# kanyu369/ADNM-UNet

Hardware: AMD Instinct MI355X
Metric: sequences/sec training ADNM-UNet 5->20x128x128 (higher is better)
Workload: dtype bf16; 1 GPU; ADNM-UNet create_ADNMUNet(5,20,6) 128x128 full training step (fwd + enRainfallLoss + bwd + clip_grad_norm_ + AdamW), recipe parameters, synthetic radar frames in HBM; per_gpu_batch=4, global_batch=4, frames=5->20, parallelism=single, launch=hipGraph replay

## Files before the change

### adnm-unet_amd/csrc/planar.hip

```cpp
#include "adnm_common.h"

namespace {

constexpr int kBlock = 256;

__device__ __forceinline__ float4 f4zero() { return make_float4(0.f, 0.f, 0.f, 0.f); }

template <typename T, int CX>
__global__ __launch_bounds__(kBlock) void haar_dwt_kernel(const T* __restrict__ x, int64_t ldx, T* __restrict__ y, int B, int H,
                                                          int W, int C) {
  const int C4 = C >> 2, h2 = (H + 1) >> 1, w2 = (W + 1) >> 1;
  const int64_t total = (int64_t)B * h2 * w2 * C4;
  const int64_t idx = (int64_t)blockIdx.x * kBlock + threadIdx.x;
  if (idx >= total) return;
  const int cg = (int)(idx % C4);
  int64_t t = idx / C4;
  const int j = (int)(t % w2);
  t /= w2;
  const int i = (int)(t % h2);
  const int b = (int)(t / h2);
  float v[4][4];
#pragma unroll
  for (int q = 0; q < 4; ++q) {
    const int hh = 2 * i + (q >> 1), ww = 2 * j + (q & 1);
// ... 348 lines not shown
                                                                    int cgb, int ppc, int act) {
  __shared__ __attribute__((aligned(16))) float smem[3 * 2 * 64 * 4];
  const int C4 = C >> 2;
  const int cgl = threadIdx.x & (cgb - 1), slot = threadIdx.x / cgb, slots = kBlock / cgb;
  const int cg = blockIdx.x * cgb + cgl;
  const bool cv = cg < C4;
  const int c = cv ? cg * 4 : 0;
  const int b = blockIdx.z;
  const T* xb = x + (int64_t)b * HW * C + c;
  const T* db = dy + (int64_t)b * HW * C + c;
  const float4 mu = *reinterpret_cast<const float4*>(mu_in + (int64_t)b * C + c);
  const float4 rs = *reinterpret_cast<const float4*>(rstd_in + (int64_t)b * C + c);
  const float sc = scale ? *scale : 1.f, sh = shift ? *shift : 0.f;
  float4 acc[2] = {f4zero(), f4zero()};
  const int64_t p0 = (int64_t)blockIdx.y * ppc;
  const int64_t p1 = p0 + ppc < HW ? p0 + ppc : HW;
  if (cv)
    for (int64_t p = p0 + slot; p < p1; p += slots) {
      const float4 v = Io<T>::ld4(xb + p * C), g = Io<T>::ld4(db + p * C);
      const float4 xh = make_float4((v.x - mu.x) * rs.x, (v.y - mu.y) * rs.y, (v.z - mu.z) * rs.z, (v.w - mu.w) * rs.w);
      const float4 ag = actg4(make_float4(sc * xh.x + sh, sc * xh.y + sh, sc * xh.z + sh, sc * xh.w + sh), act);
      const float4 dp = make_float4(g.x * ag.x, g.y * ag.y, g.z * ag.z, g.w * ag.w);
      acc[0].x += dp.x; acc[0].y += dp.y; acc[0].z += dp.z; acc[0].w += dp.w;
      acc[1].x = fmaf(dp.x, xh.x, acc[1].x); acc[1].y = fmaf(dp.y, xh.y, acc[1].y);
      acc[1].z = fmaf(dp.z, xh.z, acc[1].z); acc[1].w = fmaf(dp.w, xh.w, acc[1].w);
    }
  fold_slots<2>(acc, cgb, smem);
  if ((threadIdx.x >> 6) == 0) {
    const bool mine = (threadIdx.x & 63) < cgb && cv;
    if (mine) {
      float* dst = part + ((int64_t)b * gridDim.y + blockIdx.y) * 2 * C;
      *reinterpret_cast<float4*>(dst + c) = acc[0];
      *reinterpret_cast<float4*>(dst + C + c) = acc[1];
    }
    if (spart) {
      float a = mine ? (acc[0].x + acc[0].y) + (acc[0].z + acc[0].w) : 0.f, q = mine ? (acc[1].x + acc[1].y) + (acc[1].z + acc[1].w) : 0.f;
      a = wave_sum(a), q = wave_sum(q);
      if (threadIdx.x == 0) {
        float* sp = spart + (((int64_t)b * gridDim.y + blockIdx.y) * gridDim.x + blockIdx.x) * 2;
        sp[0] = a, sp[1] = q;
      }
    }
  }
}

template <typename T>
__global__ __launch_bounds__(kBlock) void instnorm_bwd_apply_kernel(const T* __restrict__ dy, const T* __restrict__ x,
                                                                    const float* __restrict__ part, const float* __restrict__ scale,
                                                                    const float* __restrict__ shift, const float* __restrict__ mu_in,
                                                                    const float* __restrict__ rstd_in, T* __restrict__ dx, int64_t HW,
                                                                    int C, int cgb, int ppc, int nchunk, int act) {
  const int C4 = C >> 2;
  const int cgl = threadIdx.x & (cgb - 1), slot = threadIdx.x / cgb, slots = kBlock / cgb;
  const int cg = blockIdx.x * cgb + cgl;
  const bool cv = cg < C4;
  const int c = cv ? cg * 4 : 0;
  const int b = blockIdx.z;
  float4 s1, s2;
  merge_partials(part, b, nchunk, C, c, cv, cgb, s1, s2);
  if (!cv) return;
  const T* xb = x + (int64_t)b * HW * C + c;
  const T* db = dy + (int64_t)b * HW * C + c;
  T* ob = dx + (int64_t)b * HW * C + c;
  const float4 mu = *reinterpret_cast<const float4*>(mu_in + (int64_t)b * C + c);
  const float4 rs = *reinterpret_cast<const float4*>(rstd_in + (int64_t)b * C + c);
  const float sc = scale ? *scale : 1.f, sh = shift ? *shift : 0.f;
  const float inv = 1.0f / (float)HW;
  s1.x *= inv; s1.y *= inv; s1.z *= inv; s1.w *= inv;
  s2.x *= inv; s2.y *= inv; s2.z *= inv; s2.w *= inv;
  const int64_t p0 = (int64_t)blockIdx.y * ppc;
  const int64_t p1 = p0 + ppc < HW ? p0 + ppc : HW;
  for (int64_t p = p0 + slot; p < p1; p += slots) {
    const float4 v = Io<T>::ld4(xb + p * C), g = Io<T>::ld4(db + p * C);
    const float4 xh = make_float4((v.x - mu.x) * rs.x, (v.y - mu.y) * rs.y, (v.z - mu.z) * rs.z, (v.w - mu.w) * rs.w);
    const float4 ag = actg4(make_float4(sc * xh.x + sh, sc * xh.y + sh, sc * xh.z + sh, sc * xh.w + sh), act);
    float4 o;
    o.x = rs.x * sc * (g.x * ag.x - s1.x - xh.x * s2.x);
    o.y = rs.y * sc * (g.y * ag.y - s1.y - xh.y * s2.y);
    o.z = rs.z * sc * (g.z * ag.z - s1.z - xh.z * s2.z);
    o.w = rs.w * sc * (g.w * ag.w - s1.w - xh.w * s2.w);
    Io<T>::st4(ob + p * C, o);
  }
}



__device__ __forceinline__ float hsum4(float4 v) { return (v.x + v.y) + (v.z + v.w); }
__device__ __forceinline__ float dot4(float4 a, float4 b) { return (a.x * b.x + a.y * b.y) + (a.z * b.z + a.w * b.w); }
__device__ __forceinline__ float4 ld4_or(const float* p, int c, float dflt) {
  return p ? *reinterpret_cast<const float4*>(p + c) : make_float4(dflt, dflt, dflt, dflt);
}

__device__ __forceinline__ void group_sums(float h1, float h2, const float* __restrict__ part, const float* __restrict__ w, int b,
                                           int nchunk, int C, int c, bool cv, int cgb, int cpg, float& g1, float& g2) {
  __shared__ float gsm[2][64];
  if (threadIdx.x < cgb) gsm[0][threadIdx.x] = h1, gsm[1][threadIdx.x] = h2;
  __syncthreads();
  g1 = g2 = 0.f;
  if (!cv) return;
  const int qpg = cpg >> 2, q0 = c / cpg * qpg, base = blockIdx.x * cgb;
  if (q0 >= base && q0 + qpg <= base + cgb) {
    for (int q = q0 - base; q < q0 - base + qpg; ++q) g1 += gsm[0][q], g2 += gsm[1][q];
  } else {
    for (int q = q0; q < q0 + qpg; ++q) {
      float4 a = f4zero(), s = f4zero();
      for (int k = 0; k < nchunk; ++k) {
        const float* src = part + ((int64_t)b * nchunk + k) * 2 * C + q * 4;
        const float4 ak = *reinterpret_cast<const float4*>(src), sk = *reinterpret_cast<const float4*>(src + C);
        a.x += ak.x; a.y += ak.y; a.z += ak.z; a.w += ak.w;
        s.x += sk.x; s.y += sk.y; s.z += sk.z; s.w += sk.w;
      }
      const float4 wq = ld4_or(w, q * 4, 1.f);
      g1 += dot4(wq, a), g2 += dot4(wq, s);
    }
  }
}

template <typename T>
__global__ __launch_bounds__(kBlock) void groupnorm_apply_kernel(const T* __restrict__ x, const float* __restrict__ part,
                                                                 const float* __restrict__ gamma, const float* __restrict__ beta,
                                                                 const float* __restrict__ scale, const float* __restrict__ shift,
                                                                 T* __restrict__ y, float* __restrict__ mu_out, float* __restrict__ rstd_out,
                                                                 int64_t HW, int C, int cpg, int cgb, int ppc, int nchunk, float eps, int act) {
  const int C4 = C >> 2;
  const int cgl = threadIdx.x & (cgb - 1), slot = threadIdx.x / cgb, slots = kBlock / cgb;
  const int cg = blockIdx.x * cgb + cgl;
  const bool cv = cg < C4;
  const int c = cv ? cg * 4 : 0;
  const int b = blockIdx.z;
  float4 s1, s2;
  merge_partials(part, b, nchunk, C, c, cv, cgb, s1, s2);
  float g1, g2;
  group_sums(hsum4(s1), hsum4(s2), part, nullptr, b, nchunk, C, c, cv, cgb, cpg, g1, g2);
  if (!cv) return;
  const T* xb = x + (int64_t)b * HW * C + c;
  T* yb = y + (int64_t)b * HW * C + c;
  const float K = Io<T>::ld(xb - c % cpg);
  const float inv = 1.0f / ((float)HW * (float)cpg);
  const float m = g1 * inv;
  const float rstd = rsqrtf(fmaxf(g2 * inv - m * m, 0.f) + eps);
  if (blockIdx.y == 0 && slot == 0 && c % cpg == 0) {
    const int64_t at = (int64_t)b * (C / cpg) + c / cpg;
    mu_out[at] = K + m;
    rstd_out[at] = rstd;
  }
  const float sc = scale ? *scale : 1.f, sh = shift ? *shift : 0.f;
  const float4 ga = ld4_or(gamma, c, 1.f), be = ld4_or(beta, c, 0.f);
  const float4 a = make_float4(sc * ga.x * rstd, sc * ga.y * rstd, sc * ga.z * rstd, sc * ga.w * rstd);
  const float4 o0 = make_float4(fmaf(sc, be.x, sh), fmaf(sc, be.y, sh), fmaf(sc, be.z, sh), fmaf(sc, be.w, sh));
  const int64_t p0 = (int64_t)blockIdx.y * ppc;
  const int64_t p1 = p0 + ppc < HW ? p0 + ppc : HW;
  for (int64_t p = p0 + slot; p < p1; p += slots) {
    const float4 v = Io<T>::ld4(xb + p * C);
    float4 o = make_float4(fmaf((v.x - K) - m, a.x, o0.x), fmaf((v.y - K) - m, a.y, o0.y), fmaf((v.z - K) - m, a.z, o0.z),
                           fmaf((v.w - K) - m, a.w, o0.w));
    Io<T>::st4(yb + p * C, act4(o, act));
  }
}

template <typename T>
__global__ __launch_bounds__(kBlock) void groupnorm_bwd_stats_kernel(const T* __restrict__ dy, const T* __restrict__ x,
                                                                     const float* __restrict__ gamma, const float* __restrict__ beta,
                                                                     const float* __restrict__ scale, const float* __restrict__ shift,
                                                                     const float* __restrict__ mu_in, const float* __restrict__ rstd_in,
                                                                     float* __restrict__ part, float* __restrict__ spart, int64_t HW, int C,
                                                                     int cpg, int cgb, int ppc, int act) {
// ... 110 lines not shown

extern "C" int adnm_haar_idwt(const void* s, const void* up1, const void* up2, const void* ll_add, const void* y_add1, const void* y_add2, void* y,
                              int64_t B, int64_t H, int64_t W, int64_t C, int dtype, adnm_stream_t stream) {
  ADNM_REQUIRE(s && y, "haar_idwt: null pointer");
  ADNM_REQUIRE(up1 || !up2, "haar_idwt: the coarser levels must be filled in order (up2 without up1)");
  ADNM_REQUIRE(B > 0 && H > 0 && W > 0 && C > 0 && C % 4 == 0, "haar_idwt: bad shape (C=%lld must be a multiple of 4)", (long long)C);
  ADNM_REQUIRE(dtype == ADNM_F32 || dtype == ADNM_BF16, "haar_idwt: bad dtype %d", dtype);
  const int64_t total = B * ((H + 1) / 2) * ((W + 1) / 2) * (C / 4);
  const unsigned grid = (unsigned)adnm_cdiv(total, kBlock);
  hipStream_t st = (hipStream_t)stream;
  const double units = 2.0 + (up1 ? 0.25 : 0.0) + (up2 ? 0.0625 : 0.0) + (ll_add ? (up2 ? 0.015625 : (up1 ? 0.0625 : 0.25)) : 0.0) + (y_add1 ? 1.0 : 0.0) + (y_add2 ? 1.0 : 0.0);
  const int up = up2 ? 2 : (up1 ? 1 : 0);
#define IDWT(T, UP) haar_idwt_kernel<T, UP><<<grid, kBlock, 0, st>>>((const T*)s, (const T*)up1, (const T*)up2, (const T*)ll_add, (const T*)y_add1, (const T*)y_add2, (T*)y, (int)B, (int)H, (int)W, (int)C)
  if (dtype == ADNM_F32) {
    ADNM_PROF("haar_idwt", st, 4.0 * B * H * W * C * units);
    if (up == 0) IDWT(float, 0);
    else if (up == 1) IDWT(float, 1);
    else IDWT(float, 2);
  } else {
    ADNM_PROF("haar_idwt", st, 2.0 * B * H * W * C * units);
    if (up == 0) IDWT(uint16_t, 0);
    else if (up == 1) IDWT(uint16_t, 1);
    else IDWT(uint16_t, 2);
  }
#undef IDWT
  ADNM_CHECK_LAUNCH("haar_idwt");
  return ADNM_OK;
}

static int pool_geo(const char* who, int64_t B, int64_t H, int64_t W, int64_t C, int kh, int kw, int stride, int dtype, PoolGeo* g) {
  ADNM_REQUIRE(B > 0 && H > 0 && W > 0 && C > 0 && C % 4 == 0, "%s: bad shape (C=%lld must be a multiple of 4)", who, (long long)C);
  ADNM_REQUIRE(dtype == ADNM_F32 || dtype == ADNM_BF16, "%s: bad dtype %d", who, dtype);
  if (stride == 1) {
    ADNM_REQUIRE((kh == 1 || kh == 3) && (kw == 1 || kw == 3), "%s: stride-1 pooling supports 1x3, 3x1, 3x3 ('same' padding)", who);
    *g = PoolGeo{kh, kw, 1, kh / 2, kw / 2, (int)H, (int)W};
  } else {
    ADNM_REQUIRE(stride == kh && stride == kw && stride >= 2 && stride <= 4, "%s: strided pooling needs kernel == stride in [2,4]", who);
    *g = PoolGeo{kh, kw, stride, 0, 0, (int)(H / stride), (int)(W / stride)};
    ADNM_REQUIRE(g->Ho > 0 && g->Wo > 0, "%s: input smaller than the window", who);
  }
  return ADNM_OK;
}

extern "C" int adnm_maxpool_fwd(const void* x, void* y, int64_t B, int64_t H, int64_t W, int64_t C, int kh, int kw, int stride, int dtype,
                                adnm_stream_t stream) {
  ADNM_REQUIRE(x && y, "maxpool_fwd: null pointer");
  PoolGeo g;
  if (int rc = pool_geo("maxpool_fwd", B, H, W, C, kh, kw, stride, dtype, &g)) return rc;
  const int64_t total = B * g.Ho * g.Wo * (C / 4);
  const unsigned grid = (unsigned)adnm_cdiv(total, kBlock);
  hipStream_t st = (hipStream_t)stream;
  const double es = dtype == ADNM_F32 ? 4.0 : 2.0;
  ADNM_PROF("maxpool_fwd", st, es * C * B * ((double)H * W + (double)g.Ho * g.Wo));
  if (dtype == ADNM_F32) maxpool_fwd_kernel<float><<<grid, kBlock, 0, st>>>((const float*)x, (float*)y, (int)B, (int)H, (int)W, (int)C, g);
  else maxpool_fwd_kernel<uint16_t><<<grid, kBlock, 0, st>>>((const uint16_t*)x, (uint16_t*)y, (int)B, (int)H, (int)W, (int)C, g);
  ADNM_CHECK_LAUNCH("maxpool_fwd");
  return ADNM_OK;
}

extern "C" int adnm_maxpool_bwd(const void* dy, const void* x, const void* dx_add, void* dx, int64_t B, int64_t H, int64_t W, int64_t C, int kh, int kw, int stride,
                                int dtype, adnm_stream_t stream) {
  ADNM_REQUIRE(dy && x && dx, "maxpool_bwd: null pointer");
  PoolGeo g;
  if (int rc = pool_geo("maxpool_bwd", B, H, W, C, kh, kw, stride, dtype, &g)) return rc;
  const int64_t total = B * H * W * (C / 4);
  const unsigned grid = (unsigned)adnm_cdiv(total, kBlock);
  hipStream_t st = (hipStream_t)stream;
  const double es = dtype == ADNM_F32 ? 4.0 : 2.0;
  ADNM_PROF("maxpool_bwd", st, es * C * B * ((dx_add ? 3.0 : 2.0) * H * W + (double)g.Ho * g.Wo));
  if (dtype == ADNM_F32)
    maxpool_bwd_kernel<float><<<grid, kBlock, 0, st>>>((const float*)dy, (const float*)x, (const float*)dx_add, (float*)dx, (int)B, (int)H, (int)W, (int)C, g);
  else
    maxpool_bwd_kernel<uint16_t><<<grid, kBlock, 0, st>>>((const uint16_t*)dy, (const uint16_t*)x, (const uint16_t*)dx_add, (uint16_t*)dx, (int)B, (int)H, (int)W, (int)C, g);
  ADNM_CHECK_LAUNCH("maxpool_bwd");
  return ADNM_OK;
}

extern "C" int64_t adnm_instnorm_ws_bytes(int64_t B, int64_t HW, int64_t C) {
  if (B <= 0 || HW <= 0 || C < 4) return 0;
  const IGeo g = igeo(HW, C);
  return (B * g.nchunk * 2 * C + B * g.nchunk * (int64_t)g.gx * 2) * (int64_t)sizeof(float);
}

static int instnorm_check(const char* who, int64_t B, int64_t HW, int64_t C, int act, int dtype, void* ws, int64_t ws_bytes) {
  ADNM_REQUIRE(B > 0 && HW > 1 && C > 0 && C % 4 == 0 && B <= 65535, "%s: bad shape B=%lld HW=%lld C=%lld", who, (long long)B, (long long)HW,
               (long long)C);
  ADNM_REQUIRE(act == ADNM_ACT_NONE || act == ADNM_ACT_GELU || act == ADNM_ACT_SILU, "%s: bad activation %d", who, act);
  ADNM_REQUIRE(dtype == ADNM_F32 || dtype == ADNM_BF16, "%s: bad dtype %d", who, dtype);
  if (!ws || ws_bytes < adnm_instnorm_ws_bytes(B, HW, C)) {
    adnm_set_error("%s: workspace %lld < %lld bytes", who, (long long)ws_bytes, (long long)adnm_instnorm_ws_bytes(B, HW, C));
    return ADNM_EWORKSPACE;
  }
  return ADNM_OK;
}

extern "C" int adnm_instnorm_fwd(const void* x, const float* scale, const float* shift, void* y, float* mu, float* rstd, void* ws,
                                 int64_t ws_bytes, int64_t B, int64_t HW, int64_t C, float eps, int act, int dtype, adnm_stream_t stream) {
  ADNM_REQUIRE(x && y && mu && rstd, "instnorm_fwd: null pointer");
  if (int rc = instnorm_check("instnorm_fwd", B, HW, C, act, dtype, ws, ws_bytes)) return rc;
  const IGeo g = igeo(HW, C);
  const dim3 grid(g.gx, g.nchunk, (unsigned)B);
  hipStream_t st = (hipStream_t)stream;
  float* part = (float*)ws;
  if (dtype == ADNM_F32) {
    { ADNM_PROF("instnorm_stats", st, 4.0 * B * HW * C); instnorm_stats_kernel<float><<<grid, kBlock, 0, st>>>((const float*)x, part, HW, (int)C, g.cgb, g.pix_per_chunk); }
    { ADNM_PROF("instnorm_apply", st, 4.0 * B * HW * C * 2); instnorm_apply_kernel<float><<<grid, kBlock, 0, st>>>((const float*)x, part, scale, shift, (float*)y, mu, rstd, HW, (int)C, g.cgb,
                                                          g.pix_per_chunk, g.nchunk, eps, act); }
  } else {
    { ADNM_PROF("instnorm_stats", st, 2.0 * B * HW * C); instnorm_stats_kernel<uint16_t><<<grid, kBlock, 0, st>>>((const uint16_t*)x, part, HW, (int)C, g.cgb, g.pix_per_chunk); }
    { ADNM_PROF("instnorm_apply", st, 2.0 * B * HW * C * 2); instnorm_apply_kernel<uint16_t><<<grid, kBlock, 0, st>>>((const uint16_t*)x, part, scale, shift, (uint16_t*)y, mu, rstd, HW, (int)C,
                                                             g.cgb, g.pix_per_chunk, g.nchunk, eps, act); }
  }
  ADNM_CHECK_LAUNCH("instnorm_fwd");
  return ADNM_OK;
}

extern "C" int adnm_instnorm_bwd(const void* dy, const void* x, const float* scale, const float* shift, const float* mu,
                                 const float* rstd, void* dx, float* dscale, float* dshift, void* ws, int64_t ws_bytes, int64_t B,
                                 int64_t HW, int64_t C, int act, int dtype, adnm_stream_t stream) {
  ADNM_REQUIRE(dy && x && mu && rstd && dx, "instnorm_bwd: null pointer");
  if (int rc = instnorm_check("instnorm_bwd", B, HW, C, act, dtype, ws, ws_bytes)) return rc;
  const IGeo g = igeo(HW, C);
  const dim3 grid(g.gx, g.nchunk, (unsigned)B);
  hipStream_t st = (hipStream_t)stream;
  float* part = (float*)ws;
  float* spart = (dscale || dshift) ? part + B * g.nchunk * 2 * C : nullptr;
  if (dtype == ADNM_F32) {
    { ADNM_PROF("instnorm_bwd_stats", st, 4.0 * B * HW * C * 2); instnorm_bwd_stats_kernel<float><<<grid, kBlock, 0, st>>>((const float*)dy, (const float*)x, scale, shift, mu, rstd, part, spart, HW, (int)C,
                                                              g.cgb, g.pix_per_chunk, act); }
    { ADNM_PROF("instnorm_bwd_apply", st, 4.0 * B * HW * C * 3); instnorm_bwd_apply_kernel<float><<<grid, kBlock, 0, st>>>((const float*)dy, (const float*)x, part, scale, shift, mu, rstd, (float*)dx,
                                                              HW, (int)C, g.cgb, g.pix_per_chunk, g.nchunk, act); }
  } else {
    { ADNM_PROF("instnorm_bwd_stats", st, 2.0 * B * HW * C * 2); instnorm_bwd_stats_kernel<uint16_t><<<grid, kBlock, 0, st>>>((const uint16_t*)dy, (const uint16_t*)x, scale, shift, mu, rstd, part, spart, HW,
                                                                 (int)C, g.cgb, g.pix_per_chunk, act); }
    { ADNM_PROF("instnorm_bwd_apply", st, 2.0 * B * HW * C * 3); instnorm_bwd_apply_kernel<uint16_t><<<grid, kBlock, 0, st>>>((const uint16_t*)dy, (const uint16_t*)x, part, scale, shift, mu, rstd,
                                                                 (uint16_t*)dx, HW, (int)C, g.cgb, g.pix_per_chunk, g.nchunk, act); }
  }
  ADNM_CHECK_LAUNCH("instnorm_bwd");
  if (spart) adnm_launch_fold("instnorm_bwd_scalar", spart, (int)(B * g.nchunk * g.gx), 2, {dshift, 1}, {dscale, 1}, {nullptr, 0}, {nullptr, 0}, st);
  ADNM_CHECK_LAUNCH("instnorm_bwd");
  return ADNM_OK;
}

extern "C" int64_t adnm_groupnorm_ws_bytes(int64_t B, int64_t HW, int64_t C, int64_t G) {
  if (G <= 0 || C % G) return 0;
  return adnm_instnorm_ws_bytes(B, HW, C);
}

static int groupnorm_check(const char* who, int64_t B, int64_t HW, int64_t C, int64_t G, int act, int dtype, void* ws, int64_t ws_bytes) {
  ADNM_REQUIRE(B > 0 && HW > 0 && C > 0 && C % 4 == 0 && B <= 65535 && C <= (1 << 24), "%s: bad shape B=%lld HW=%lld C=%lld", who, (long long)B,
               (long long)HW, (long long)C);
  ADNM_REQUIRE(G > 0 && C % G == 0, "%s: %lld groups do not divide %lld channels", who, (long long)G, (long long)C);
  ADNM_REQUIRE((C / G) % 4 == 0, "%s: %lld channels per group (C=%lld, G=%lld): must be a multiple of 4 channels per group (a lane's channel quad lies inside one group)",
               who, (long long)(C / G), (long long)C, (long long)G);
  ADNM_REQUIRE(act == ADNM_ACT_NONE || act == ADNM_ACT_GELU || act == ADNM_ACT_SILU, "%s: bad activation %d", who, act);
  ADNM_REQUIRE(dtype == ADNM_F32 || dtype == ADNM_BF16, "%s: bad dtype %d", who, dtype);
  if (!ws || ws_bytes < adnm_groupnorm_ws_bytes(B, HW, C, G)) {
    adnm_set_error("%s: workspace %lld < %lld bytes", who, (long long)ws_bytes, (long long)adnm_groupnorm_ws_bytes(B, HW, C, G));
    return ADNM_EWORKSPACE;
  }
  return ADNM_OK;
}

extern "C" int adnm_groupnorm_fwd(const void* x, const float* gamma, const float* beta, const float* scale, const float* shift, void* y,
                                  float* mu, float* rstd, void* ws, int64_t ws_bytes, int64_t B, int64_t HW, int64_t C, int64_t G, float eps,
                                  int act, int dtype, adnm_stream_t stream) {
  ADNM_REQUIRE(x && y && mu && rstd, "groupnorm_fwd: null pointer");
  if (int rc = groupnorm_check("groupnorm_fwd", B, HW, C, G, act, dtype, ws, ws_bytes)) return rc;
  const IGeo g = igeo(HW, C);
  const dim3 grid(g.gx, g.nchunk, (unsigned)B);
  hipStream_t st = (hipStream_t)stream;
  float* part = (float*)ws;
  const int cpg = (int)(C / G);
  const double es = dtype == ADNM_F32 ? 4.0 : 2.0;
  if (dtype == ADNM_F32) {
    { ADNM_PROF("groupnorm_stats", st, es * B * HW * C); groupnorm_stats_kernel<float><<<grid, kBlock, 0, st>>>((const float*)x, part, HW, (int)C, cpg, g.cgb, g.pix_per_chunk); }
    { ADNM_PROF("groupnorm_apply", st, es * B * HW * C * 2); groupnorm_apply_kernel<float><<<grid, kBlock, 0, st>>>((const float*)x, part, gamma, beta, scale, shift, (float*)y, mu, rstd, HW,
                                                            (int)C, cpg, g.cgb, g.pix_per_chunk, g.nchunk, eps, act); }
  } else {
    { ADNM_PROF("groupnorm_stats", st, es * B * HW * C); groupnorm_stats_kernel<uint16_t><<<grid, kBlock, 0, st>>>((const uint16_t*)x, part, HW, (int)C, cpg, g.cgb, g.pix_per_chunk); }
    { ADNM_PROF("groupnorm_apply", st, es * B * HW * C * 2); groupnorm_apply_kernel<uint16_t><<<grid, kBlock, 0, st>>>((const uint16_t*)x, part, gamma, beta, scale, shift, (uint16_t*)y, mu, rstd,
                                                               HW, (int)C, cpg, g.cgb, g.pix_per_chunk, g.nchunk, eps, act); }
  }
  ADNM_CHECK_LAUNCH("groupnorm_fwd");
  return ADNM_OK;
}

extern "C" int adnm_groupnorm_bwd(const void* dy, const void* x, const float* gamma, const float* beta, const float* scale, const float* shift,
                                  const float* mu, const float* rstd, void* dx, float* dgamma, float* dbeta, float* dscale, float* dshift,
                                  void* ws, int64_t ws_bytes, int64_t B, int64_t HW, int64_t C, int64_t G, int act, int dtype,
                                  adnm_stream_t stream) {
  ADNM_REQUIRE(dy && x && mu && rstd && dx, "groupnorm_bwd: null pointer");
  if (int rc = groupnorm_check("groupnorm_bwd", B, HW, C, G, act, dtype, ws, ws_bytes)) return rc;
  const IGeo g = igeo(HW, C);
  const dim3 grid(g.gx, g.nchunk, (unsigned)B);
  hipStream_t st = (hipStream_t)stream;
  float* part = (float*)ws;
  float* spart = (dscale || dshift) ? part + B * g.nchunk * 2 * C : nullptr;
  const int cpg = (int)(C / G);
  const double es = dtype == ADNM_F32 ? 4.0 : 2.0;
  if (dtype == ADNM_F32) {
    { ADNM_PROF("groupnorm_bwd_stats", st, es * B * HW * C * 2); groupnorm_bwd_stats_kernel<float><<<grid, kBlock, 0, st>>>((const float*)dy, (const float*)x, gamma, beta, scale, shift, mu, rstd, part,
                                                                spart, HW, (int)C, cpg, g.cgb, g.pix_per_chunk, act); }
    { ADNM_PROF("groupnorm_bwd_apply", st, es * B * HW * C * 3); groupnorm_bwd_apply_kernel<float><<<grid, kBlock, 0, st>>>((const float*)dy, (const float*)x, part, gamma, beta, scale, shift, mu, rstd,
                                                                (float*)dx, HW, (int)C, cpg, g.cgb, g.pix_per_chunk, g.nchunk, act); }
  } else {
    { ADNM_PROF("groupnorm_bwd_stats", st, es * B * HW * C * 2); groupnorm_bwd_stats_kernel<uint16_t><<<grid, kBlock, 0, st>>>((const uint16_t*)dy, (const uint16_t*)x, gamma, beta, scale, shift, mu, rstd,
                                                                   part, spart, HW, (int)C, cpg, g.cgb, g.pix_per_chunk, act); }
    { ADNM_PROF("groupnorm_bwd_apply", st, es * B * HW * C * 3); groupnorm_bwd_apply_kernel<uint16_t><<<grid, kBlock, 0, st>>>((const uint16_t*)dy, (const uint16_t*)x, part, gamma, beta, scale, shift, mu,
                                                                   rstd, (uint16_t*)dx, HW, (int)C, cpg, g.cgb, g.pix_per_chunk, g.nchunk, act); }
  }
  ADNM_CHECK_LAUNCH("groupnorm_bwd");
  if (dgamma || dbeta) adnm_launch_fold("groupnorm_bwd_affine", part, (int)(B * g.nchunk), (int)(2 * C), {dbeta, (int)C}, {dgamma, (int)C}, {nullptr, 0}, {nullptr, 0}, st);
  if (spart) adnm_launch_fold("groupnorm_bwd_scalar", spart, (int)(B * g.nchunk * g.gx), 2, {dshift, 1}, {dscale, 1}, {nullptr, 0}, {nullptr, 0}, st);
  ADNM_CHECK_LAUNCH("groupnorm_bwd");
  return ADNM_OK;
}
```

### include/adnm_hip.h

```cpp
#ifndef ADNM_HIP_H
#define ADNM_HIP_H

#include <stdint.h>
#include <stddef.h>

#ifdef __cplusplus
extern "C" {
#endif

typedef void* adnm_stream_t;

enum { ADNM_F32 = 0, ADNM_BF16 = 1 };
enum { ADNM_ACT_NONE = 0, ADNM_ACT_SILU = 1, ADNM_ACT_GELU = 2 };
enum { ADNM_OK = 0, ADNM_EINVAL = -1, ADNM_ELAUNCH = -2, ADNM_EWORKSPACE = -3 };
enum { ADNM_MFMA_F32 = 0, ADNM_MFMA_BF16 = 1, ADNM_MFMA_FP8 = 2, ADNM_MFMA_FP8_GRAD = 3 };
enum { ADNM_B_F32 = 0, ADNM_B_BF16 = 1, ADNM_B_FP8 = 2 };

int adnm_quant_update(float* table, int64_t n, float* state, float headroom, adnm_stream_t stream);

const char* adnm_last_error(void);
int adnm_abi_version(void);

int adnm_prof_enable(int on);
int64_t adnm_prof_collect(char* buf, int64_t buflen);

void* adnm_foldq_create(void);
int adnm_foldq_destroy(void* q);
int adnm_foldq_bind(void* q);
int64_t adnm_foldq_pending(void* q);
int adnm_foldq_flush(void* q, adnm_stream_t stream);
int adnm_foldq_clear(void* q);
int adnm_foldq_accumulate_next(int mask);

void* adnm_leafq_create(void);
int adnm_leafq_destroy(void* q);
int adnm_leafq_bind(void* q);
int64_t adnm_leafq_pending(void* q);
int adnm_leafq_flush(void* q, adnm_stream_t stream);
int adnm_leafq_clear(void* q);

int adnm_rownorm_fwd(const void* x, int64_t ldx, const float* w, const float* b, const float* scale,
                     const float* shift, void* y, int64_t ldy, float* mu, float* rstd, int64_t M, int64_t d,
                     float eps, int subtract_mean, int dtype, adnm_stream_t stream);
int64_t adnm_rownorm_bwd_ws_bytes(int64_t M, int64_t d);
int adnm_rownorm_bwd(const void* dy, int64_t lddy, const void* x, int64_t ldx, const float* w, const float* b,
                     const float* scale, const float* mu, const float* rstd, void* dx, int64_t lddx, float* dw,
                     float* db, float* dscale, float* dshift, const void* dres, int64_t lddres, void* ws, int64_t ws_bytes,
                     int64_t M, int64_t d, int subtract_mean, int dtype, adnm_stream_t stream);

int64_t adnm_ssd_ws_bytes(int64_t B, int64_t L, int64_t H, int64_t P, int64_t N, int64_t G);
int adnm_ssd_reduce_fwd(const void* x, int64_t ldx, const void* Bm, int64_t ldb, const void* Cm, int64_t ldc,
                        const void* dt_raw, int64_t lddt, int64_t dt_hstride, const float* dt_bias,
                        const float* A_log, const float* D, int64_t p_hstride, void* y, int64_t ldy, float* kv,
                        const float* ln_w, const float* ln_b, void* yn, int64_t ldyn, float* ln_mu, float* ln_rstd,
                        float ln_eps, void* ws, int64_t ws_bytes, int64_t B, int64_t L, int64_t H, int64_t P, int64_t N,
                        int64_t G, int dtype, adnm_stream_t stream);
int adnm_ssd_reduce_bwd(const void* dy, int64_t lddy, const void* x, int64_t ldx, const void* Bm, int64_t ldb,
                        const void* Cm, int64_t ldc, const void* dt_raw, int64_t lddt, int64_t dt_hstride,
                        const float* dt_bias, const float* A_log, const float* D, int64_t p_hstride,
                        const float* kv, void* dx, int64_t lddx, void* dBm, int64_t lddb, void* dCm, int64_t lddc,
                        void* ddt_raw, int64_t ldddt, float* ddt_bias, float* dA_log, float* dD, void* ws,
                        int64_t ws_bytes, int64_t B, int64_t L, int64_t H, int64_t P, int64_t N, int64_t G,
                        int dtype, adnm_stream_t stream);

int64_t adnm_ssd_scan_ws_bytes(int64_t B, int64_t L, int64_t H, int64_t N, int64_t chunk, int backward);
int adnm_ssd_scan_fwd(const void* x, int64_t ldx, int64_t x_hstride, const void* Bm, int64_t ldb, const void* Cm,
                      int64_t ldc, const void* dt_raw, int64_t lddt, int64_t dt_hstride, const float* dt_bias,
                      const float* A_log, const float* D, int64_t p_hstride, void* y, int64_t ldy, int64_t y_hstride,
                      float* S_in, void* ws, int64_t ws_bytes, int64_t B, int64_t L, int64_t H, int64_t P, int64_t N,
                      int64_t G, int64_t chunk, int reverse, int dtype, adnm_stream_t stream);
int adnm_ssd_scan_bwd(const void* dy, int64_t lddy, int64_t dy_hstride, const void* x, int64_t ldx, int64_t x_hstride,
                      const void* Bm, int64_t ldb, const void* Cm, int64_t ldc, const void* dt_raw, int64_t lddt,
                      int64_t dt_hstride, const float* dt_bias, const float* A_log, const float* D, int64_t p_hstride,
                      const float* S_in, void* dx, int64_t lddx, int64_t dx_hstride, void* dBm, int64_t lddb, void* dCm,
                      int64_t lddc, void* ddt_raw, int64_t ldddt, int64_t ddt_hstride, float* ddt_bias, float* dA_log,
                      float* dD, void* ws, int64_t ws_bytes, int64_t B, int64_t L, int64_t H, int64_t P, int64_t N,
                      int64_t G, int64_t chunk, int reverse, int dtype, adnm_stream_t stream);

int adnm_dwconv_fwd(const void* x, int64_t ldx, const float* wgt, const float* bias, const void* addend,
                    int64_t ldadd, void* y, int64_t ldy, int64_t B, int64_t H, int64_t W, int64_t C, int KH,
                    int KW, int act, int wlayout, int dtype, adnm_stream_t stream);
int64_t adnm_dwconv_bwd_ws_bytes(int64_t B, int64_t H, int64_t W, int64_t C, int KH, int KW);
int adnm_dwconv_bwd(const void* dy, int64_t lddy, const void* x, int64_t ldx, const float* wgt,
                    const float* bias, void* dpre, void* dx, int64_t lddx, float* dwgt, float* dbias, void* ws,
                    int64_t ws_bytes, int64_t B, int64_t H, int64_t W, int64_t C, int KH, int KW, int act,
                    int wlayout, int dtype, adnm_stream_t stream);
int adnm_dwconv_wgrad(const void* g, int64_t ldg, const void* x, int64_t ldx, float* dwgt, float* dbias, void* ws, int64_t ws_bytes,
                      int64_t B, int64_t H, int64_t W, int64_t C, int KH, int KW, int wlayout, int dtype, adnm_stream_t stream);

int adnm_haar_dwt(const void* x, int64_t ldx, int64_t cx, void* y, int64_t B, int64_t H, int64_t W, int64_t C,
                  int dtype, adnm_stream_t stream);
int adnm_wt_level(const float* x, int64_t ldx, int64_t cx, const float* taps, float* sub, float* tag, int64_t B, int64_t H, int64_t W,
                  int64_t C, int K, int flip, adnm_stream_t stream);
int adnm_haar_idwt(const void* s, const void* up1, const void* up2, const void* ll_add, const void* y_add1, const void* y_add2, void* y,
                   int64_t B, int64_t H, int64_t W, int64_t C, int dtype, adnm_stream_t stream);

int adnm_maxpool_fwd(const void* x, void* y, int64_t B, int64_t H, int64_t W, int64_t C, int kh, int kw, int stride,
                     int dtype, adnm_stream_t stream);
int adnm_maxpool_bwd(const void* dy, const void* x, const void* dx_add, void* dx, int64_t B, int64_t H, int64_t W, int64_t C, int kh,
                     int kw, int stride, int dtype, adnm_stream_t stream);

int64_t adnm_instnorm_ws_bytes(int64_t B, int64_t HW, int64_t C);
int adnm_instnorm_fwd(const void* x, const float* scale, const float* shift, void* y, float* mu, float* rstd,
                      void* ws, int64_t ws_bytes, int64_t B, int64_t HW, int64_t C, float eps, int act, int dtype,
                      adnm_stream_t stream);
int adnm_instnorm_bwd(const void* dy, const void* x, const float* scale, const float* shift, const float* mu,
                      const float* rstd, void* dx, float* dscale, float* dshift, void* ws, int64_t ws_bytes,
                      int64_t B, int64_t HW, int64_t C, int act, int dtype, adnm_stream_t stream);

int64_t adnm_groupnorm_ws_bytes(int64_t B, int64_t HW, int64_t C, int64_t G);
int adnm_groupnorm_fwd(const void* x, const float* gamma, const float* beta, const float* scale, const float* shift, void* y,
                       float* mu, float* rstd, void* ws, int64_t ws_bytes, int64_t B, int64_t HW, int64_t C, int64_t G, float eps,
                       int act, int dtype, adnm_stream_t stream);
int adnm_groupnorm_bwd(const void* dy, const void* x, const float* gamma, const float* beta, const float* scale, const float* shift,
                       const float* mu, const float* rstd, void* dx, float* dgamma, float* dbeta, float* dscale, float* dshift,
                       void* ws, int64_t ws_bytes, int64_t B, int64_t HW, int64_t C, int64_t G, int act, int dtype,
                       adnm_stream_t stream);

int adnm_gate_fwd(const void* h, int64_t ldh, void* y, int64_t ldy, int64_t M, int64_t F, int dtype,
                  adnm_stream_t stream);
int adnm_gate_bwd(const void* dy, int64_t lddy, const void* h, int64_t ldh, void* dh, int64_t lddh, int64_t M,
                  int64_t F, int dtype, adnm_stream_t stream);

int adnm_igate_fwd(const void* x, const float* enhance, const float* threshold, void* y, int64_t n, int dtype,
                   adnm_stream_t stream);
int64_t adnm_igate_bwd_ws_bytes(int64_t n);
int adnm_igate_bwd(const void* dy, const void* x, const float* enhance, const float* threshold, void* dx, float* denhance,
                   float* dthreshold, void* ws, int64_t ws_bytes, int64_t n, int dtype, adnm_stream_t stream);
int adnm_igate_res_fwd(const float* x, const float* res, int per_token, const float* gama, const float* enhance,
                       const float* threshold, float* y, int64_t B, int64_t L, int64_t C, adnm_stream_t stream);
int64_t adnm_igate_res_bwd_ws_bytes(int64_t B, int64_t L, int64_t C);
int adnm_igate_res_bwd(const float* dy, const float* x, const float* res, int per_token, const float* gama, const float* enhance,
                       const float* threshold, float* dx, float* dres, float* dgama, float* denhance, float* dthreshold, void* ws,
                       int64_t ws_bytes, int64_t B, int64_t L, int64_t C, adnm_stream_t stream);


int adnm_skipgate_fwd(const float* x, const float* const* params, float* pooled, float* conv, float* out, int64_t B, int64_t H, int64_t W,
                      int64_t C, adnm_stream_t stream);
int64_t adnm_skipgate_grad_floats(int64_t C);
int64_t adnm_skipgate_bwd_ws_bytes(int64_t B, int64_t H, int64_t W, int64_t C);
int adnm_skipgate_bwd(const float* dout, const float* x, const float* const* params, const float* pooled, const float* conv, float* dx,
                      float* dparams, void* ws, int64_t ws_bytes, int64_t B, int64_t H, int64_t W, int64_t C, adnm_stream_t stream);

int adnm_attn4_fwd(const float* qkv, float* out, float* lse, int64_t B, int64_t L, int64_t heads, float scale, adnm_stream_t stream);
int adnm_attn4_bwd(const float* dout, const float* qkv, const float* out, const float* lse, float* dqkv, int64_t B, int64_t L, int64_t heads,
                   float scale, adnm_stream_t stream);

int adnm_emul_fwd(const float* a, int64_t lda, const float* b, int64_t ldb, float* y, int64_t M, int64_t C, adnm_stream_t stream);
int adnm_emul_bwd(const float* dy, const float* a, int64_t lda, const float* b, int64_t ldb, float* da, float* db, int64_t M, int64_t C,
                  adnm_stream_t stream);
int adnm_chancopy(const float* x, int64_t ldx, int64_t Cin, float* y, int64_t Cout, int64_t M, adnm_stream_t stream);
int adnm_conv1d3_fwd(const float* x, const float* w, const float* bias, float* y, int64_t B, int64_t n, adnm_stream_t stream);
int adnm_conv1d3_bwd(const float* dy, const float* x, const float* w, float* dx, float* dwb, int64_t B, int64_t n, adnm_stream_t stream);
int adnm_bridge_heads_fwd(const float* att, const float* const* W, const float* const* bias, const int64_t* C, int nheads,
                          const float* enhance, const float* threshold, float* const* z, float* const* y, int64_t B, int64_t S,
                          adnm_stream_t stream);
int64_t adnm_bridge_heads_bwd_ws_bytes(int64_t total, int64_t B, int64_t S);
int adnm_bridge_heads_bwd(const float* att, const float* const* W, const int64_t* C, int nheads, const float* enhance,
                          const float* threshold, const float* const* z, const float* const* dy, float* datt, float* const* dW,
                          float* const* dbias, float* denhance, float* dthreshold, void* ws, int64_t ws_bytes, int64_t B, int64_t S,
                          adnm_stream_t stream);

int64_t adnm_bridge_pool_ws_bytes(int64_t B, int64_t S);
int adnm_bridge_pool_fwd(int64_t n, const float* const* x, const int64_t* L, const int64_t* C, float* att, void* ws, int64_t ws_bytes, int64_t B,
                         adnm_stream_t stream);
int adnm_bridge_pool_bwd(int64_t n, const float* const* dxa, const float* datt, const int64_t* L, const int64_t* C, float* const* dx, int64_t B,
                         adnm_stream_t stream);

int64_t adnm_colsum_ws_bytes(int64_t rows, int64_t n);
int adnm_colsum(const float* x, float* out, int64_t rows, int64_t n, void* ws, int64_t ws_bytes, adnm_stream_t stream);

#define ADNM_SKGEMM_NT 0
#define ADNM_SKGEMM_NN 1
#define ADNM_SKGEMM_TN 2
int adnm_skgemm_supported(int op, int64_t M, int64_t N, int64_t K);
int64_t adnm_skgemm_ws_bytes(int op, int64_t M, int64_t N, int64_t K);
int adnm_skgemm(int op, const float* a, int64_t lda, const void* b, int64_t ldb, int b_dtype, const float* b_scale, const float* bias, float* c,
                int64_t ldc, float* dbias, void* ws, int64_t ws_bytes, void* slabs_uc, int64_t slabs_uc_bytes, int64_t M, int64_t N, int64_t K,
                int prec, float* q, adnm_stream_t stream);
int64_t adnm_skgemm_counter_bytes(int op, int64_t M, int64_t N, int64_t K);
void* adnm_uncached_alloc(int64_t bytes);
int adnm_uncached_free(void* ptr);

int64_t adnm_rainloss_ws_bytes(int64_t n);
int adnm_rainloss(const float* pred, const float* target, float* loss, float* grad, void* ws, int64_t ws_bytes, int64_t n, float omega_t,
// ... 106 lines not shown
```

Baseline: 498.8 sequences/s.

## Fuse instance-norm stats and apply into single-pass register-resident kernels

Adds one-pass forward and backward instance-norm kernels. Each block owns a channel group across the entire spatial extent, holds the inputs in registers (up to 16 rows per thread), reduces the statistics in shared memory and applies the normalization without reading the input a second time. This replaces the previous two-kernel stats+apply scheme and its global partial-sum workspace whenever the plane fits the register budget. The trade-off is that the grid no longer splits over spatial chunks, so parallelism is lower, and register pressure is higher. An environment variable can disable the path.

```diff
diff --git a/adnm-unet_amd/csrc/planar.hip b/adnm-unet_amd/csrc/planar.hip
--- a/adnm-unet_amd/csrc/planar.hip
+++ b/adnm-unet_amd/csrc/planar.hip
@@ -454,6 +454,189 @@
     Io<T>::st4(ob + p * C, o);
   }
 }
+
+struct OGeo {
+  int cgb, gx, R;
+};
+OGeo ogeo(int64_t HW, int64_t C, int dtype) {
+  static const bool on = [] { const char* e = getenv("ADNM_INSTNORM_ONEPASS"); return !e || atoi(e) != 0; }();
+  OGeo g;
+  const int64_t C4 = C / 4;
+  const int full = dtype == ADNM_F32 ? 4 : 8, rmax = 16;
+  g.cgb = 1;
+  while (g.cgb < full && g.cgb < C4) g.cgb <<= 1;
+  if (g.cgb == 8 && HW * 8 > (int64_t)kBlock * rmax) g.cgb = 4;
+  g.gx = (int)adnm_cdiv(C4, g.cgb);
+  g.R = 1;
+  while (g.R <= rmax && HW * g.cgb > (int64_t)kBlock * g.R) g.R <<= 1;
+  if (g.R > rmax || !on || HW * C >= ((int64_t)1 << 31)) g.R = 0;
+  return g;
+}
+
+template <typename T>
+struct Quad;
+template <>
+struct Quad<float> {
+  typedef float4 type;
+  static __device__ __forceinline__ float4 ld(const float* p) { return *reinterpret_cast<const float4*>(p); }
+  static __device__ __forceinline__ float4 f4(float4 q) { return q; }
+  static __device__ __forceinline__ void keep(float4&) {}
+};
+template <>
+struct Quad<uint16_t> {
+  typedef uint2 type;
+  static __device__ __forceinline__ uint2 ld(const uint16_t* p) { return *reinterpret_cast<const uint2*>(p); }
+  static __device__ __forceinline__ float4 f4(uint2 r) {
+    return make_float4(__uint_as_float(r.x << 16), __uint_as_float(r.x & 0xffff0000u), __uint_as_float(r.y << 16), __uint_as_float(r.y & 0xffff0000u));
+  }
+  static __device__ __forceinline__ void keep(uint2& q) { asm volatile("" : "+v"(q.x), "+v"(q.y)); }
+};
+
+__device__ __forceinline__ void fold_publish(float4 (&acc)[2], int cgb, int cgl, float4& s1, float4& s2) {
+  __shared__ __attribute__((aligned(16))) float smem[3 * 2 * 64 * 4];
+  __shared__ __attribute__((aligned(16))) float mout[2][64][4];
+  fold_slots<2>(acc, cgb, smem);
+  if ((threadIdx.x >> 6) == 0 && (threadIdx.x & 63) < cgb) {
+    *reinterpret_cast<float4*>(&mout[0][cgl][0]) = acc[0];
+    *reinterpret_cast<float4*>(&mout[1][cgl][0]) = acc[1];
+  }
+  __syncthreads();
+  s1 = *reinterpret_cast<const float4*>(&mout[0][cgl][0]);
+  s2 = *reinterpret_cast<const float4*>(&mout[1][cgl][0]);
+}
+
+template <typename T, int R>
+__global__ __launch_bounds__(kBlock, 2) void instnorm_fwd_onepass_kernel(const T* __restrict__ x, const float* __restrict__ scale,
+                                                                      const float* __restrict__ shift, T* __restrict__ y,
+                                                                      float* __restrict__ mu_out, float* __restrict__ rstd_out, int HW, int C,
+                                                                      int cgb, float eps, int act) {
+  const int C4 = C >> 2;
+  const int cgl = threadIdx.x & (cgb - 1), slot = threadIdx.x / cgb, slots = kBlock / cgb;
+  const int cg = blockIdx.x * cgb + cgl;
+  const bool cv = cg < C4;
+  const int c = cv ? cg * 4 : 0;
+  const int b = blockIdx.z;
+  const T* xb = x + (int64_t)b * HW * C;
+  T* yb = y + (int64_t)b * HW * C;
+  const unsigned off = (unsigned)slot * C + c, step = (unsigned)slots * C;
+  typename Quad<T>::type xq[R];
+#pragma unroll
+  for (int r = 0; r < R; ++r) xq[r] = cv && slot + r * slots < HW ? Quad<T>::ld(xb + (size_t)r * step + off) : Quad<T>::ld(xb + c);
+  const float4 K = Io<T>::ld4(xb + c);
+  float4 acc[2] = {f4zero(), f4zero()};
+#pragma unroll
+  for (int r = 0; r < R; ++r) {
+    const float4 v = Quad<T>::f4(xq[r]);
+    const float d0 = v.x - K.x, d1 = v.y - K.y, d2 = v.z - K.z, d3 = v.w - K.w;
+    acc[0].x += d0; acc[0].y += d1; acc[0].z += d2; acc[0].w += d3;
+    acc[1].x = fmaf(d0, d0, acc[1].x); acc[1].y = fmaf(d1, d1, acc[1].y);
+    acc[1].z = fmaf(d2, d2, acc[1].z); acc[1].w = fmaf(d3, d3, acc[1].w);
+  }
+  float4 s1, s2;
+  fold_publish(acc, cgb, cgl, s1, s2);
+  if (!cv) return;
+  const float inv = 1.0f / (float)HW;
+  const float4 m = make_float4(s1.x * inv, s1.y * inv, s1.z * inv, s1.w * inv);
+  const float4 mu = make_float4(K.x + m.x, K.y + m.y, K.z + m.z, K.w + m.w);
+  float4 rstd;
+  rstd.x = rsqrtf(fmaxf(s2.x * inv - m.x * m.x, 0.f) + eps);
+  rstd.y = rsqrtf(fmaxf(s2.y * inv - m.y * m.y, 0.f) + eps);
+  rstd.z = rsqrtf(fmaxf(s2.z * inv - m.z * m.z, 0.f) + eps);
+  rstd.w = rsqrtf(fmaxf(s2.w * inv - m.w * m.w, 0.f) + eps);
+  if (slot == 0) {
+    *reinterpret_cast<float4*>(mu_out + (int64_t)b * C + c) = mu;
+    *reinterpret_cast<float4*>(rstd_out + (int64_t)b * C + c) = rstd;
+  }
+  const float sc = scale ? *scale : 1.f, sh = shift ? *shift : 0.f;
+#pragma unroll
+  for (int r = 0; r < R; ++r) {
+    if (slot + r * slots < HW) {
+      Quad<T>::keep(xq[r]);
+      const float4 v = Quad<T>::f4(xq[r]);
+      float4 o = make_float4(sc * (v.x - mu.x) * rstd.x + sh, sc * (v.y - mu.y) * rstd.y + sh, sc * (v.z - mu.z) * rstd.z + sh,
+                             sc * (v.w - mu.w) * rstd.w + sh);
+      Io<T>::st4(yb + (size_t)r * step + off, act4(o, act));
+    }
+  }
+}
+
+template <typename T, int R>
+__global__ __launch_bounds__(kBlock, 2) void instnorm_bwd_onepass_kernel(const T* __restrict__ dy, const T* __restrict__ x,
+                                                                      const float* __restrict__ scale, const float* __restrict__ shift,
+                                                                      const float* __restrict__ mu_in, const float* __restrict__ rstd_in,
+                                                                      T* __restrict__ dx, float* __restrict__ spart, int HW, int C, int cgb,
+                                                                      int act) {
+  const int C4 = C >> 2;
+  const int cgl = threadIdx.x & (cgb - 1), slot = threadIdx.x / cgb, slots = kBlock / cgb;
+  const int cg = blockIdx.x * cgb + cgl;
+  const bool cv = cg < C4;
+  const int c = cv ? cg * 4 : 0;
+  const int b = blockIdx.z;
+  const T* xb = x + (int64_t)b * HW * C;
+  const T* db = dy + (int64_t)b * HW * C;
+  T* ob = dx + (int64_t)b * HW * C;
+  const unsigned off = (unsigned)slot * C + c, step = (unsigned)slots * C;
+  typename Quad<T>::type xq[R];
+  float4 dp[R];
+#pragma unroll
+  for (int r = 0; r < R; ++r) {
+    const bool in = cv && slot + r * slots < HW;
+    xq[r] = in ? Quad<T>::ld(xb + (size_t)r * step + off) : Quad<T>::ld(xb + c);
+    dp[r] = in ? Io<T>::ld4(db + (size_t)r * step + off) : f4zero();
+  }
+  const float4 mu = *reinterpret_cast<const float4*>(mu_in + (int64_t)b * C + c);
+  const float4 rs = *reinterpret_cast<const float4*>(rstd_in + (int64_t)b * C + c);
+  const float sc = scale ? *scale : 1.f, sh = shift ? *shift : 0.f;
+  float4 acc[2] = {f4zero(), f4zero()};
+#pragma unroll
+  for (int r = 0; r < R; ++r) {
+    const float4 v = Quad<T>::f4(xq[r]);
+    const float4 xh = make_float4((v.x - mu.x) * rs.x, (v.y - mu.y) * rs.y, (v.z - mu.z) * rs.z, (v.w - mu.w) * rs.w);
+    const float4 ag = actg4(make_float4(sc * xh.x + sh, sc * xh.y + sh, sc * xh.z + sh, sc * xh.w + sh), act);
+    dp[r] = make_float4(dp[r].x * ag.x, dp[r].y * ag.y, dp[r].z * ag.z, dp[r].w * ag.w);
+    acc[0].x += dp[r].x; acc[0].y += dp[r].y; acc[0].z += dp[r].z; acc[0].w += dp[r].w;
+    acc[1].x = fmaf(dp[r].x, xh.x, acc[1].x); acc[1].y = fmaf(dp[r].y, xh.y, acc[1].y);
+    acc[1].z = fmaf(dp[r].z, xh.z, acc[1].z); acc[1].w = fmaf(dp[r].w, xh.w, acc[1].w);
+  }
+  float4 s1, s2;
+  fold_publish(acc, cgb, cgl, s1, s2);
+  if (spart && (threadIdx.x >> 6) == 0) {
+    const bool mine = (threadIdx.x & 63) < cgb && cv;
+    float a = mine ? (acc[0].x + acc[0].y) + (acc[0].z + acc[0].w) : 0.f, q = mine ? (acc[1].x + acc[1].y) + (acc[1].z + acc[1].w) : 0.f;
+    a = wave_sum(a), q = wave_sum(q);
+    if (threadIdx.x == 0) {
+      float* sp = spart + ((int64_t)b * gridDim.x + blockIdx.x) * 2;
+      sp[0] = a, sp[1] = q;
+    }
+  }
+  if (!cv) return;
+  const float inv = 1.0f / (float)HW;
+  s1.x *= inv; s1.y *= inv; s1.z *= inv; s1.w *= inv;
+  s2.x *= inv; s2.y *= inv; s2.z *= inv; s2.w *= inv;
+#pragma unroll
+  for (int r = 0; r < R; ++r) {
+    if (slot + r * slots < HW) {
+      Quad<T>::keep(xq[r]);
+      const float4 v = Quad<T>::f4(xq[r]);
+      const float4 xh = make_float4((v.x - mu.x) * rs.x, (v.y - mu.y) * rs.y, (v.z - mu.z) * rs.z, (v.w - mu.w) * rs.w);
+      float4 o;
+      o.x = rs.x * sc * (dp[r].x - s1.x - xh.x * s2.x);
+      o.y = rs.y * sc * (dp[r].y - s1.y - xh.y * s2.y);
+      o.z = rs.z * sc * (dp[r].z - s1.z - xh.z * s2.z);
+      o.w = rs.w * sc * (dp[r].w - s1.w - xh.w * s2.w);
+      Io<T>::st4(ob + (size_t)r * step + off, o);
+    }
+  }
+}
+
+#define ADNM_ONEPASS_R(R_, LAUNCH)   \
+  switch (R_) {                      \
+    case 1: { LAUNCH(1); } break;    \
+    case 2: { LAUNCH(2); } break;    \
+    case 4: { LAUNCH(4); } break;    \
+    case 8: { LAUNCH(8); } break;    \
+    default: { LAUNCH(16); } break;  \
+  }
 
 
 
@@ -730,6 +913,11 @@
   return (B * g.nchunk * 2 * C + B * g.nchunk * (int64_t)g.gx * 2) * (int64_t)sizeof(float);
 }
 
+extern "C" int adnm_instnorm_onepass(int64_t HW, int64_t C, int dtype) {
+  if (HW <= 1 || C < 4 || C % 4 || (dtype != ADNM_F32 && dtype != ADNM_BF16)) return 0;
+  return ogeo(HW, C, dtype).R;
+}
+
 static int instnorm_check(const char* who, int64_t B, int64_t HW, int64_t C, int act, int dtype, void* ws, int64_t ws_bytes) {
   ADNM_REQUIRE(B > 0 && HW > 1 && C > 0 && C % 4 == 0 && B <= 65535, "%s: bad shape B=%lld HW=%lld C=%lld", who, (long long)B, (long long)HW,
                (long long)C);
@@ -750,7 +938,17 @@
   const dim3 grid(g.gx, g.nchunk, (unsigned)B);
   hipStream_t st = (hipStream_t)stream;
   float* part = (float*)ws;
-  if (dtype == ADNM_F32) {
+  const OGeo o = ogeo(HW, C, dtype);
+  if (o.R) {
+    const dim3 ogrid(o.gx, 1, (unsigned)B);
+    ADNM_PROF("instnorm_apply", st, (dtype == ADNM_F32 ? 4.0 : 2.0) * B * HW * C * 2);
+#define LAUNCH(R_) instnorm_fwd_onepass_kernel<float, R_><<<ogrid, kBlock, 0, st>>>((const float*)x, scale, shift, (float*)y, mu, rstd, (int)HW, (int)C, o.cgb, eps, act)
+    if (dtype == ADNM_F32) ADNM_ONEPASS_R(o.R, LAUNCH)
+#undef LAUNCH
+#define LAUNCH(R_) instnorm_fwd_onepass_kernel<uint16_t, R_><<<ogrid, kBlock, 0, st>>>((const uint16_t*)x, scale, shift, (uint16_t*)y, mu, rstd, (int)HW, (int)C, o.cgb, eps, act)
+    else ADNM_ONEPASS_R(o.R, LAUNCH)
+#undef LAUNCH
+  } else if (dtype == ADNM_F32) {
     { ADNM_PROF("instnorm_stats", st, 4.0 * B * HW * C); instnorm_stats_kernel<float><<<grid, kBlock, 0, st>>>((const float*)x, part, HW, (int)C, g.cgb, g.pix_per_chunk); }
     { ADNM_PROF("instnorm_apply", st, 4.0 * B * HW * C * 2); instnorm_apply_kernel<float><<<grid, kBlock, 0, st>>>((const float*)x, part, scale, shift, (float*)y, mu, rstd, HW, (int)C, g.cgb,
                                                           g.pix_per_chunk, g.nchunk, eps, act); }
@@ -773,7 +971,20 @@
   hipStream_t st = (hipStream_t)stream;
   float* part = (float*)ws;
   float* spart = (dscale || dshift) ? part + B * g.nchunk * 2 * C : nullptr;
-  if (dtype == ADNM_F32) {
+  int64_t srows = B * g.nchunk * g.gx;
+  const OGeo o = ogeo(HW, C, dtype);
+  if (o.R) {
+    const dim3 ogrid(o.gx, 1, (unsigned)B);
+    if (spart) spart = part;
+    srows = B * o.gx;
+    ADNM_PROF("instnorm_bwd_apply", st, (dtype == ADNM_F32 ? 4.0 : 2.0) * B * HW * C * 3);
+#define LAUNCH(R_) instnorm_bwd_onepass_kernel<float, R_><<<ogrid, kBlock, 0, st>>>((const float*)dy, (const float*)x, scale, shift, mu, rstd, (float*)dx, spart, (int)HW, (int)C, o.cgb, act)
+    if (dtype == ADNM_F32) ADNM_ONEPASS_R(o.R, LAUNCH)
+#undef LAUNCH
+#define LAUNCH(R_) instnorm_bwd_onepass_kernel<uint16_t, R_><<<ogrid, kBlock, 0, st>>>((const uint16_t*)dy, (const uint16_t*)x, scale, shift, mu, rstd, (uint16_t*)dx, spart, (int)HW, (int)C, o.cgb, act)
+    else ADNM_ONEPASS_R(o.R, LAUNCH)
+#undef LAUNCH
+  } else if (dtype == ADNM_F32) {
     { ADNM_PROF("instnorm_bwd_stats", st, 4.0 * B * HW * C * 2); instnorm_bwd_stats_kernel<float><<<grid, kBlock, 0, st>>>((const float*)dy, (const float*)x, scale, shift, mu, rstd, part, spart, HW, (int)C,
                                                               g.cgb, g.pix_per_chunk, act); }
     { ADNM_PROF("instnorm_bwd_apply", st, 4.0 * B * HW * C * 3); instnorm_bwd_apply_kernel<float><<<grid, kBlock, 0, st>>>((const float*)dy, (const float*)x, part, scale, shift, mu, rstd, (float*)dx,
@@ -785,7 +996,7 @@
                                                                  (uint16_t*)dx, HW, (int)C, g.cgb, g.pix_per_chunk, g.nchunk, act); }
   }
   ADNM_CHECK_LAUNCH("instnorm_bwd");
-  if (spart) adnm_launch_fold("instnorm_bwd_scalar", spart, (int)(B * g.nchunk * g.gx), 2, {dshift, 1}, {dscale, 1}, {nullptr, 0}, {nullptr, 0}, st);
+  if (spart) adnm_launch_fold("instnorm_bwd_scalar", spart, (int)srows, 2, {dshift, 1}, {dscale, 1}, {nullptr, 0}, {nullptr, 0}, st);
   ADNM_CHECK_LAUNCH("instnorm_bwd");
   return ADNM_OK;
 }
diff --git a/include/adnm_hip.h b/include/adnm_hip.h
--- a/include/adnm_hip.h
+++ b/include/adnm_hip.h
@@ -101,6 +101,7 @@
                      int kw, int stride, int dtype, adnm_stream_t stream);
 
 int64_t adnm_instnorm_ws_bytes(int64_t B, int64_t HW, int64_t C);
+int adnm_instnorm_onepass(int64_t HW, int64_t C, int dtype);
 int adnm_instnorm_fwd(const void* x, const float* scale, const float* shift, void* y, float* mu, float* rstd,
                       void* ws, int64_t ws_bytes, int64_t B, int64_t HW, int64_t C, float eps, int act, int dtype,
                       adnm_stream_t stream);
```

Measured after the change: 500.4 sequences/s, median of 6. About the same (+0.3%).
